# kpreid/all-is-cubes

Measured on NVIDIA H100. Metric: Mrays/s, higher is better.
Workload: dtype f64 geometry / f32 colour

## Files before the change

### all-is-cubes_b200/aicb200/__init__.py

```python
from __future__ import annotations

import ctypes as C
import dataclasses
import math
import os
from typing import Optional, Sequence

import numpy as np

from . import abi
from .abi import (FOG_ABRUPT, FOG_COMPROMISE, FOG_NONE, FOG_PHYSICAL, LIGHT_BOUNCE, LIGHT_COARSE, LIGHT_FLAT, LIGHT_LINEAR,
                  LIGHT_NONE, LIGHT_SMOOTHSTEP, TONE_CLAMP, TONE_REINHARD, TRANSPARENCY_SURFACE,
                  TRANSPARENCY_THRESHOLD, TRANSPARENCY_VOLUMETRIC)

PKG_DIR = os.path.dirname(os.path.dirname(os.path.abspath(__file__)))
LIB_PATH = os.environ.get("AICB200_LIB") or os.path.join(PKG_DIR, "libaicb200.so")
LIGHT_RAY_DTYPE = np.dtype(abi.LightRay)


class AicbError(RuntimeError):
    def __init__(self, status: int, message: str):
        super().__init__(f"{abi.STATUS_NAMES.get(status, status)}: {message}")
        self.status = status

# ... 787 lines not shown
    for c in rgb:
        f = np.float32(c) / np.float32(255.0)
        if f <= np.float32(0.04045):
            out.append(float(np.float32(f * np.float32(25.0 / 323.0))))
        else:
            x = np.float32(np.float32(200.0) * f + np.float32(11.0)) / np.float32(211.0)
            out.append(float(np.float32(float(x) ** float(np.float32(12.0 / 5.0)))))
    return tuple(out)


class Context:
    _default = None

    def __init__(self, device_id: int = -1):
        lib = load_library()
        self.handle = C.c_void_p()
        _check(lib.aicb_ctx_create(device_id, C.byref(self.handle)))
        self.device_id = lib.aicb_ctx_device(self.handle)
        self._pending = None

    def settle(self):
        if self._pending is not None:
            self._pending.result()

    @classmethod
    def default(cls) -> "Context":
        if cls._default is None:
            cls._default = Context(-1)
        return cls._default

    def derive_block_light(self, blocks: Sequence[Block]) -> list:
        if not blocks:
            return []
        descs = _block_descs(blocks)
        out = (abi.BlockLight * len(blocks))()
        _check(load_library().aicb_derive_block_light(self.handle, descs, len(blocks), out))
        return [BlockLight.from_abi(o) for o in out]

    def close(self):
        if self.handle:
            load_library().aicb_ctx_destroy(self.handle)
            self.handle = C.c_void_p()


@dataclasses.dataclass
class RenderInfo:
    cubes_traced: int
    rays: int
    algorithmic_bytes: int
    counters: tuple
    kernel_ms: float
    flaws: int
    stage_ms: tuple = (0.0, 0.0, 0.0, 0.0)

    @staticmethod
    def from_abi(i: abi.RenderInfo) -> "RenderInfo":
        return RenderInfo(int(i.cubes_traced), int(i.rays), int(i.algorithmic_bytes), tuple(int(c) for c in i.counters),
                          float(i.kernel_ms), int(i.flaws), tuple(float(v) for v in i.stage_ms))


@dataclasses.dataclass
class Rendering:
    size: tuple
    data: np.ndarray
    flaws: int
    info: RenderInfo


def _torch():
    import torch
    return torch


def _ctx_device(ctx: "Context"):
    return _torch().device("cuda", ctx.device_id)


def _device_outputs(out, device, spec) -> dict:
    torch = _torch()
    given = out if isinstance(out, dict) else ({next(iter(spec)): out} if out is not None else {})
    unknown = set(given) - set(spec)
    if unknown:
        raise ValueError(f"out= names outputs this call does not make: {sorted(unknown)}")
    tensors = {}
    for name, (shape, dtype) in spec.items():
        t = given.get(name)
        if t is None:
            t = torch.empty(shape, dtype=dtype, device=device)
        elif tuple(t.shape) != tuple(shape) or t.dtype != dtype or t.device != device or not t.is_contiguous():
            raise ValueError(f"out[{name!r}] must be a contiguous {dtype} tensor of shape {tuple(shape)} on {device}, "
                             f"not {t.dtype} {tuple(t.shape)} on {t.device}")
        tensors[name] = t
    return tensors


def _outs_abi(n: int, tensors: dict) -> abi.DeviceOutputs:
    o = abi.DeviceOutputs()
    for name, t in tensors.items():
        setattr(o, name, t.data_ptr())
    o.len = n
    return o


def _stream(device) -> int:
    return _torch().cuda.current_stream(device).cuda_stream or 1


class DeviceRendering:

    def __init__(self, scene, issue, build):
        self._scene = scene
# ... 1180 lines not shown
```

### all-is-cubes_b200/aicb200/abi.py

```python
import ctypes as C

import numpy as np

ABI_VERSION = 27

BLOCKS_DERIVE_LIGHT = 1

OK, ERR_INVALID, ERR_OOM, ERR_CUDA, ERR_UNSUPPORTED, ERR_BUSY, ERR_RETRY = range(7)
STATUS_NAMES = {0: "OK", 1: "ERR_INVALID", 2: "ERR_OOM", 3: "ERR_CUDA", 4: "ERR_UNSUPPORTED", 5: "ERR_BUSY", 6: "ERR_RETRY"}

FACE_WITHIN, FACE_NX, FACE_NY, FACE_NZ, FACE_PX, FACE_PY, FACE_PZ = range(7)
FOG_NONE, FOG_ABRUPT, FOG_COMPROMISE, FOG_PHYSICAL = range(4)
LIGHT_NONE, LIGHT_FLAT, LIGHT_COARSE, LIGHT_LINEAR, LIGHT_SMOOTHSTEP, LIGHT_BOUNCE = range(6)
TRANSPARENCY_SURFACE, TRANSPARENCY_VOLUMETRIC, TRANSPARENCY_THRESHOLD = range(3)
TONE_CLAMP, TONE_REINHARD = range(2)


class Aab(C.Structure):
    _fields_ = [("lower", C.c_int32 * 3), ("size", C.c_uint32 * 3)]


class Voxel(C.Structure):
    _fields_ = [("rgba", C.c_float * 4), ("emission", C.c_float * 3), ("flags", C.c_uint32)]

# ... 37 lines not shown
        ("block_ids", C.c_void_p),
        ("light", C.c_void_p),
        ("blocks", C.POINTER(BlockDesc)),
        ("n_blocks", C.c_size_t),
        ("sky", Sky),
        ("light_max_distance", C.c_uint8),
        ("_pad", C.c_uint8 * 7),
    ]


class CameraData(C.Structure):
    _fields_ = [
        ("inverse_projection_view", C.c_double * 16),
        ("fb_width", C.c_uint32),
        ("fb_height", C.c_uint32),
        ("exposure", C.c_float),
        ("_pad", C.c_uint32),
    ]


CAMERA_DTYPE = np.dtype([("inverse_projection_view", "<f8", (16,)), ("fb_width", "<u4"), ("fb_height", "<u4"),
                         ("exposure", "<f4"), ("_pad", "<u4")])
assert CAMERA_DTYPE.itemsize == C.sizeof(CameraData) == 144


class Options(C.Structure):
    _fields_ = [
        ("fog", C.c_uint8),
        ("lighting_display", C.c_uint8),
        ("transparency", C.c_uint8),
        ("antialiasing_always", C.c_uint8),
        ("tone_mapping", C.c_uint8),
        ("debug_pixel_cost", C.c_uint8),
        ("include_sky", C.c_uint8),
        ("bounce_samples", C.c_uint8),
        ("transparency_threshold", C.c_float),
        ("maximum_intensity", C.c_float),
        ("view_distance", C.c_double),
    ]


class Shard(C.Structure):
    _fields_ = [("strip_rows", C.c_uint32), ("index", C.c_uint32), ("count", C.c_uint32)]


class RenderInfo(C.Structure):
    _fields_ = [
        ("cubes_traced", C.c_uint64),
        ("rays", C.c_uint64),
        ("algorithmic_bytes", C.c_uint64),
        ("counters", C.c_uint64 * 6),
        ("kernel_ms", C.c_float),
        ("flaws", C.c_uint16),
        ("_pad", C.c_uint16),
        ("stage_ms", C.c_float * 4),
    ]


class Hit(C.Structure):
    _fields_ = [("cube", C.c_int32 * 3), ("voxel", C.c_int32 * 3), ("resolution", C.c_int32), ("face", C.c_int32)]


class LightRay(C.Structure):
    _fields_ = [("trigger_cube", C.c_int32 * 3), ("value_cube", C.c_int32 * 3), ("value", C.c_uint8 * 4),
                ("light_from_struck_face", C.c_float * 3), ("_pad", C.c_uint32)]


class LightUpdatesInfo(C.Structure):
    _fields_ = [("update_count", C.c_uint64), ("queue_count", C.c_uint64), ("max_update_difference", C.c_uint8),
                ("max_queue_priority", C.c_uint8), ("_pad", C.c_uint8 * 6)]


class Layer(C.Structure):
    _fields_ = [("scene", C.c_void_p), ("camera", C.POINTER(CameraData)), ("options", C.POINTER(Options))]


class GroupLayer(C.Structure):
    _fields_ = [("scene", C.c_void_p), ("camera", C.POINTER(CameraData)), ("options", C.POINTER(Options))]


TEXT_ENTERED_SPACE, TEXT_EMPTY, TEXT_INCOMPLETE, TEXT_BLANK = -1, -2, -3, -4
LAYER_NONE, LAYER_WORLD, LAYER_UI = 0, 1, 2


class TerminalPixel(C.Structure):
    _fields_ = [("rgba", C.c_float * 4), ("text", C.c_int32), ("layer", C.c_int32)]


class DeviceOutputs(C.Structure):
    _fields_ = [("srgb8", C.c_void_p), ("rgba16f", C.c_void_p), ("colorbuf", C.c_void_p), ("depth", C.c_void_p),
                ("hit", C.c_void_p), ("steps", C.c_void_p), ("text", C.c_void_p), ("texel_rgba16f", C.c_void_p),
                ("texel_depth", C.c_void_p), ("terminal", C.c_void_p), ("len", C.c_size_t), ("full_frame", C.c_uint32),
                ("_pad", C.c_uint32)]


TEXTURE_INCREMENTAL, TEXTURE_CONSISTENT = 1, 2


class TextureTargetInfo(C.Structure):
    _fields_ = [("width", C.c_uint32), ("height", C.c_uint32), ("strategy", C.c_uint32), ("_pad", C.c_uint32),
                ("dirty_pixels", C.c_uint64), ("next_pick", C.c_uint64), ("cycle_length", C.c_uint64)]


VOXEL_NOT_SELECTABLE = 1
VOXEL_NO_COLLISION = 2
BLOCK_NOT_SELECTABLE = 1
CURSOR_NONE = 0xFFFFFFFF
# ... 220 lines not shown
```

### all-is-cubes_b200/csrc/aicb200.cu

```cuda
#include <algorithm>
#include <array>
#include <cmath>
#include <cstdio>
#include <cstdlib>
#include <cstring>
#include <initializer_list>
#include <mutex>
#include <string>
#include <unordered_map>
#include <vector>

#include <cuda_runtime.h>
#include <cub/device/device_radix_sort.cuh>

#include "block_words.cuh"
#include "brick_room.h"
#include "host_tables.h"
#include "internal.h"

using namespace aicb;

static thread_local std::string g_last_error = "";

aicb_status aicb_fail(aicb_status st, const std::string &msg) {
// ... 516 lines not shown
    P.lighting = opt->lighting_display;
    P.transparency = opt->transparency;
    P.threshold = opt->transparency_threshold;
    P.antialias = (cam && opt->antialiasing_always) ? 1 : 0;
    if (cam && out.force_antialias >= 0) P.antialias = (uint32_t)out.force_antialias;
    P.tone_mapping = opt->tone_mapping;
    P.maximum_intensity = opt->maximum_intensity;
    P.view_distance = opt->view_distance;
    P.debug_pixel_cost = opt->debug_pixel_cost;
    P.include_sky = opt->include_sky;
    P.out_full_frame = out.full_frame ? 1 : 0;
    P.target = out.target;
    const int tgt = out.kind;
    if (tgt == TGT_VIEWS) P.target.view_tiles = P.tiles_x * P.tiles_y;
    P.counters = ctx->d_counters.get<unsigned long long>();
    P.task_counter = ctx->d_tile_counter;
    P.refill_threshold = REFILL_THRESHOLD;
    P.tail_divisor = TAIL_DIVISOR;
    P.event_threshold = EVENT_THRESHOLD;

    uint64_t frame_pixels = pixels, frame_rays = pixels * (P.antialias ? 4 : 1);
    uint64_t out_bytes =
        (P.target.out_srgb8 ? 4 : (tgt == TGT_TEX ? 12 : (tgt == TGT_TERM ? 24 : (P.target.out_rgba16f ? 8 : 16)))) * pixels;
    if (continues && ctx->last_scene) {
        aicb_scene *prev = ctx->last_scene;
        frame_pixels += prev->pending_pixels;
        frame_rays += prev->pending_rays;
        out_bytes += prev->pending_out_bytes;
        prev->pending = false;
    }
    sc->pending = true;
    sc->pending_pixels = frame_pixels;
    sc->pending_rays = frame_rays;
    sc->pending_out_bytes = out_bytes;

    P.n_samples = P.antialias ? 4 : 1;
    const bool fused = (opt->lighting_display == AICB_LIGHT_NONE || opt->lighting_display == AICB_LIGHT_FLAT) &&
                       !ctx->deep_frames;
    const uint64_t total_tasks = (uint64_t)P.n_tasks * P.n_samples;
    uint64_t CHUNK = (uint64_t)4 << 20;
    {
        const uint64_t per_task = sizeof(RayRecordA) + sizeof(RayRecordB) + sizeof(TaskOut) + 4 * N_BINS +
                                  (uint64_t)ctx->hits_per_task * (sizeof(HitRecord) + (fused ? 0 : sizeof(ShadedHit)));
        uint64_t fit = ((uint64_t)8 << 30) / per_task;
        if (fit < (1u << 17)) fit = 1u << 17;
        if (fit < CHUNK) CHUNK = fit & ~(uint64_t)127;
    }
    const uint64_t chunk_cap = total_tasks < CHUNK ? total_tasks : CHUNK;
    uint64_t cap = chunk_cap * ctx->hits_per_task;
    if (cap < (1u << 16)) cap = 1u << 16;
    if (cap > 0xfffffff0ull) cap = 0xfffffff0ull;
    cap &= ~(uint64_t)(HIT_CHUNK - 1);
    P.hit_capacity = (uint32_t)cap;
    TRY(ctx->primary.size(chunk_cap, P.hit_capacity, !fused));
    ctx->primary.bind(P, chunk_cap, !fused);
    P.ray_counter = ctx->d_tile_counter + 2;
    sc->pending_fused = fused;
    P.hit_counter = ctx->d_tile_counter + 1;
    P.bin_count = ctx->d_tile_counter + 4;
    P.bin_stride = (uint32_t)chunk_cap;
    P.overflow_flag = (unsigned int *)(P.counters + 7);
    if (stream != ctx->stream.get()) CU(cudaStreamWaitEvent(stream, ctx->ev_delta.get(), 0));
    if (ctx->frame_in_flight && ctx->last_stream != stream) CU(cudaStreamWaitEvent(stream, ctx->ev1.get(), 0));
    ctx->frame_in_flight = true;
    ctx->last_stream = stream;
    ctx->last_scene = sc;
    if (continues) {
        CU(cudaMemsetAsync(ctx->d_tile_counter, 0, 2 * (4 + N_BINS) * sizeof(unsigned int), stream));
    } else {
        CU(cudaMemsetAsync(P.counters, 0, 8 * sizeof(unsigned long long) + 2 * (4 + N_BINS) * sizeof(unsigned int), stream));
        CU(cudaEventRecord(ctx->ev0.get(), stream));
    }
    if (total_tasks > 0) {
        const bool volumetric = opt->transparency == AICB_TRANSPARENCY_VOLUMETRIC;
        const int lc = opt->lighting_display == AICB_LIGHT_NONE ? LC_NONE
                       : (opt->lighting_display == AICB_LIGHT_FLAT ? LC_FLAT
                          : (opt->lighting_display == AICB_LIGHT_BOUNCE ? LC_BOUNCE : LC_INTERP));
        TraceParams Q;
        const bool bounce = lc == LC_BOUNCE;
        if (bounce) {
            TRY(ctx->secondary.size(chunk_cap, P.hit_capacity, true));
            TRY(ctx->d_bounce.ensure(chunk_cap * 104 + 256));
            char *b = ctx->d_bounce.get<char>();
            P.bounce_mode = BOUNCE_PRIMARY;
            P.bounce_samples = opt->bounce_samples;
            P.bounce_rays = (double *)b;
            P.bounce_rng = (unsigned long long *)(b + chunk_cap * 48);
            P.bounce_sum = (float4 *)(b + chunk_cap * 80);
            P.bounce_req = (uint32_t *)(b + chunk_cap * 96);
            P.ray_index = (uint32_t *)(b + chunk_cap * 100);
            Q = P;
            Q.ray_index = nullptr;
            Q.bounce_mode = BOUNCE_SECONDARY;
            Q.rays = P.bounce_rays;
            Q.tiles_y = 1;
            Q.shard_count = 1; Q.shard_index = 0; Q.strip_rows = 1;
            Q.antialias = 0;
            Q.n_samples = 1;
            Q.task_base = 0;
            Q.lighting = AICB_LIGHT_FLAT;
            Q.include_sky = 1;
            Q.exposure = 1.0f;
            Q.out_full_frame = 0;
            Q.target = {};
            ctx->secondary.bind(Q, chunk_cap, true);
            Q.task_counter = ctx->d_tile_counter + (4 + N_BINS);
            Q.hit_counter = Q.task_counter + 1;
            Q.ray_counter = Q.task_counter + 2;
// ... 83 lines not shown
        float t[4] = {0, 0, 0, 0};
        for (int i = 0; i < (sc->pending_fused ? 3 : 4); i++) cudaEventElapsedTime(&t[i], ctx->ev_k[i].get(), ctx->ev_k[i + 1].get());
        if (ctx->d_debug && ctx->debug_warps) {
            std::vector<unsigned long long> w(4 * (size_t)ctx->debug_warps);
            cudaMemcpy(w.data(), ctx->d_debug.get(), w.size() * 8, cudaMemcpyDeviceToHost);
            unsigned long long t0 = ~0ull, t1 = 0, passes = 0, rays = 0;
            for (uint32_t i = 0; i < ctx->debug_warps; i++) { t0 = std::min(t0, w[4 * i]); t1 = std::max(t1, w[4 * i + 1]); passes += w[4 * i + 2]; rays += w[4 * i + 3]; }
            std::vector<double> ends;
            for (uint32_t i = 0; i < ctx->debug_warps; i++) ends.push_back((double)(w[4 * i + 1] - t0) * 1e-6);
            std::sort(ends.begin(), ends.end());
            auto q = [&](double f) { return ends[(size_t)(f * (ends.size() - 1))]; };
            fprintf(stderr, "[aicb200] march warps %u: end times ms min %.3f p10 %.3f p50 %.3f p90 %.3f p99 %.3f max %.3f; passes/warp %.0f rays %llu\n",
                    ctx->debug_warps, q(0), q(0.1), q(0.5), q(0.9), q(0.99), q(1.0), (double)passes / ctx->debug_warps, rays);
        }
        if (sc->pending_fused)
            fprintf(stderr, "[aicb200] gen %.3f ms  march %.3f ms  resolve (shade + encode) %.3f ms  (hits %llu)\n", t[0], t[1],
                    t[2], c[3]);
        else
            fprintf(stderr, "[aicb200] gen %.3f ms  march %.3f ms  shade %.3f ms  encode %.3f ms  (hits %llu)\n", t[0], t[1], t[2],
                    t[3], c[3]);
    }
    if (sc->pending_rays) ctx->deep_frames = c[3] * 4 >= sc->pending_rays * 3;
    if (c[7]) {
        if (ctx->hits_per_task >= 2048)
            return fail(AICB_ERR_OOM, "hit stream overflowed at its largest capacity (2048 hit records per ray)");
        ctx->hits_per_task *= 4;
        ctx->shallow_frames = 0;
        return fail(AICB_ERR_RETRY, "hit stream overflowed; its capacity has been raised - re-issue the render");
    }
    if (ctx->hits_per_task > 8 && c[3] * 16 < (unsigned long long)sc->pending_rays * ctx->hits_per_task) {
        if (++ctx->shallow_frames >= 16) {
            ctx->hits_per_task /= 4;
            ctx->shallow_frames = 0;
            ctx->primary.release_hits();
            ctx->secondary.release_hits();
        }
    } else {
        ctx->shallow_frames = 0;
    }
    if (info) {
        std::memset(info, 0, sizeof *info);
        float ms = 0.0f;
        CU(cudaEventElapsedTime(&ms, ctx->ev0.get(), ctx->ev1.get()));
        info->kernel_ms = ms;
        if (sc->pending_rays && ctx->stage_timing)
            for (int i = 0; i < (sc->pending_fused ? 3 : 4); i++)
                cudaEventElapsedTime(&info->stage_ms[i], ctx->ev_k[i].get(), ctx->ev_k[i + 1].get());
        info->cubes_traced = c[0];
        info->rays = sc->pending_rays;
        for (int i = 0; i < 5; i++) info->counters[i] = c[1 + i];
        info->counters[5] = sc->pending_pixels;
        info->algorithmic_bytes = 2 * c[1] + 2 * c[2] + 32 * c[3] + 4 * c[4] + 32 * c[5] + sc->pending_out_bytes;
        info->flaws = 0;
    }
    sc->pending = false;
    return AICB_OK;
}

aicb_status issue_empty_frame(aicb_scene *s, const aicb_options *opt, cudaStream_t stream) {
    return launch_trace(s, nullptr, opt, nullptr, Outputs{}, stream);
}

aicb_status check_device_pointer(const void *p, int device, bool peer_ok, size_t align, const char *what) {
    if ((uintptr_t)p % align)
        return fail(AICB_ERR_INVALID, std::string(what) + " is not aligned to " + std::to_string(align) + " bytes");
    cudaPointerAttributes a;
    const cudaError_t e = cudaPointerGetAttributes(&a, p);
    if (e != cudaSuccess) cudaGetLastError();
    if (e != cudaSuccess || (a.type != cudaMemoryTypeDevice && a.type != cudaMemoryTypeManaged))
        return fail(AICB_ERR_INVALID, std::string(what) + " is not device memory");
    if (a.device == device) return AICB_OK;
    int can = 0;
    if (peer_ok && cudaDeviceCanAccessPeer(&can, device, a.device) == cudaSuccess && can) return AICB_OK;
    return fail(AICB_ERR_INVALID, std::string(what) + " is memory of another device");
}

aicb_status output_target(const aicb_device_outputs *d, DeviceCall call, bool need_colorbuf, Outputs *o) {
    if (!d) return fail(AICB_ERR_INVALID, "outs is NULL");
    const void *const ptr[10] = {d->srgb8, d->rgba16f, d->colorbuf, d->depth, d->hit,
                                 d->steps, d->text,    d->texel_rgba16f, d->texel_depth, d->terminal};
    unsigned set = 0;
    for (int i = 0; i < 10; i++)
        if (ptr[i]) set |= 1u << i;
    const unsigned SRGB8 = 1, RGBA16F = 2, AUX = 4 | 8 | 16 | 32, TEXT = 64, TEXELS = 128 | 256, TERMINAL = 512;
    const bool aux = set && !(set & ~AUX);
    bool ok = false;
    switch (call) {
        case DEV_FRAME: ok = set == SRGB8 || set == RGBA16F || aux || set == TEXT; break;
        case DEV_RAYS: ok = aux; break;
        case DEV_LAYERS: ok = set == SRGB8 || set == TERMINAL || set == TEXELS; break;
    }
    if (set == 0 && d->len == 0) ok = true;
    if (!ok) return fail(AICB_ERR_INVALID, "the outputs are not a set that this call gives (aicb_device_outputs)");
    if (aux && need_colorbuf && d->len && !d->colorbuf) return fail(AICB_ERR_INVALID, "colorbuf is NULL");
    TargetParams &t = o->target;
    t.out_srgb8 = (uchar4 *)d->srgb8;
    t.out_text = d->text;
    o->aux = aux;
    if (aux) {
        t.out_colorbuf = (float4 *)d->colorbuf;
        t.out_depth = d->depth;
        t.out_hit = d->hit;
        t.out_steps = d->steps;
    }
    if (set == RGBA16F) t.out_rgba16f = (uint2 *)d->rgba16f;
    if (set == TEXELS) {
// ... 1777 lines not shown
    const aicb_device_outputs o = one_output(&aicb_device_outputs::text, out, out_len);
    return on_scene(s, [&](Replicas r) { return views_host(r, cameras, n_views, opt, o, STAGE_GIVEN, info); });
}

aicb_status aicb_render_views_device(aicb_scene *s, const aicb_camera *d_cameras, size_t n_views, uint32_t fb_width,
                                     uint32_t fb_height, const aicb_options *opt, const aicb_device_outputs *outs,
                                     void *stream) {
    if (!s || !outs) return fail(AICB_ERR_INVALID, "NULL argument");
    if (outs->full_frame) return fail(AICB_ERR_INVALID, "full_frame is for aicb_render_device");
    TRY(check_views(d_cameras, false, n_views, &fb_width, &fb_height, opt, outs->len));
    std::lock_guard<std::mutex> lock(s->ctx->mu);
    CU(cudaSetDevice(s->ctx->device));
    Outputs o;
    TRY(device_target(outs, s->ctx->device, DEV_FRAME, false, false, &o));
    if (n_views) TRY(check_device_pointer(d_cameras, s->ctx->device, false, 8, "the camera table"));
    cudaStream_t st = stream ? (cudaStream_t)stream : s->ctx->stream.get();
    if (outs->len == 0) return issue_empty_frame(s, opt, st);
    views_part(&o, d_cameras, n_views, 0, 1);
    const aicb_camera size = views_frame_camera(fb_width, fb_height);
    return launch_trace(s, &size, opt, nullptr, o, st);
}

aicb_status aicb_check_layers(const aicb_layer *world, const aicb_layer *ui, const float *no_world_rgba, size_t out_len,
                              const aicb_layer **lead_out) {
    const bool have_world = world && world->scene, have_ui = ui && ui->scene;
    if (!have_world && !have_ui && !no_world_rgba) return fail(AICB_ERR_INVALID, "no layer to draw");
    const aicb_layer *lead = have_world ? world : ui;
    if (!lead || !lead->camera || !lead->options) return fail(AICB_ERR_INVALID, "a layer needs its camera and options");
    if (have_ui && (!ui->camera || !ui->options)) return fail(AICB_ERR_INVALID, "a layer needs its camera and options");
    if (have_world && have_ui) {
        if (world->scene->ctx != ui->scene->ctx) return fail(AICB_ERR_INVALID, "the layers must live on one context");
        if (world->camera->fb_width != ui->camera->fb_width || world->camera->fb_height != ui->camera->fb_height)
            return fail(AICB_ERR_INVALID, "the layers' cameras must share the framebuffer size");
    }
    aicb_status st = aicb_check_render_args(lead->scene, lead->camera, lead->options, nullptr, out_len);
    if (st != AICB_OK) return st;
    if (have_ui && have_world) {
        st = validate_options(ui->options);
        if (st != AICB_OK) return st;
    }
    *lead_out = lead;
    return AICB_OK;
}

void aicb_merge_info(aicb_render_info *sum, const aicb_render_info *one, bool same_part) {
    auto time = [same_part](float t, float u) { return same_part ? t + u : std::max(t, u); };
    sum->cubes_traced += one->cubes_traced;
    sum->rays += one->rays;
    sum->algorithmic_bytes += one->algorithmic_bytes;
    for (int k = 0; k < 6; k++) sum->counters[k] += one->counters[k];
    sum->kernel_ms = time(sum->kernel_ms, one->kernel_ms);
    for (int k = 0; k < 4; k++) sum->stage_ms[k] = time(sum->stage_ms[k], one->stage_ms[k]);
    sum->flaws |= one->flaws;
}

aicb_status aicb_trace_pass(FramePart *parts, size_t n_parts, const aicb_camera *cam, const aicb_options *opt,
                            bool want_info, const std::vector<Delivery> &copies) {
    std::vector<size_t> todo(n_parts), again;
    for (size_t i = 0; i < n_parts; i++) todo[i] = i;
    while (!todo.empty()) {
        std::vector<aicb_ctx *> round = {parts[0].scene->ctx};
        for (size_t i : todo) {
            const FramePart &p = parts[i];
            aicb_ctx *ctx = p.scene->ctx;
            CU(cudaSetDevice(ctx->device));
            aicb_status r = launch_trace(p.scene, cam, opt, p.shard, p.out, ctx->stream.get());
            if (r != AICB_OK) return r;
            if (i) round.push_back(ctx);
        }
        if (!copies.empty()) TRY(deliver(round.data(), round.size(), copies));
        again.clear();
        for (size_t i : todo) {
            aicb_scene *sc = parts[i].scene;
            CU(cudaSetDevice(sc->ctx->device));
            CU(cudaStreamSynchronize(sc->ctx->stream.get()));
            aicb_render_info one{};
            aicb_status r = finish(sc, want_info ? &one : nullptr);
            if (r == AICB_ERR_RETRY) { again.push_back(i); continue; }
            if (r != AICB_OK) return r;
            aicb_merge_info(&parts[i].info, &one, true);
        }
        todo.swap(again);
    }
    return AICB_OK;
}

aicb_status aicb_trace_layers(const aicb_layer *world, const aicb_layer *ui, const float *backdrop_rgba,
                              const float *no_world_rgba, LayerPart *parts, size_t n_parts,
                              const std::vector<Delivery> &copies, aicb_render_info *total, cudaStream_t async) {
    const bool have_world = world && world->scene, have_ui = ui && ui->scene;
    const aicb_layer *lead = have_world ? world : ui;
    aicb_status st = AICB_OK;
    const int aa = lead->options->antialiasing_always ? 1 : 0;
    auto n_tasks = [&](const LayerPart &p) -> size_t {
        return (listed(p.out.target) ? (size_t)p.out.target.n_list
                                        : (((size_t)lead->camera->fb_width + TILE_W - 1) / TILE_W) *
                                              ((shard_rows(lead->camera->fb_height, &p.shard) + TILE_H - 1) / TILE_H) * 32) *
               (aa ? 4 : 1);
    };
    float backdrop[4] = {0, 0, 0, 1}, no_world[4] = {0, 0, 0, 0};
    const bool have_backdrop = backdrop_rgba && !(backdrop_rgba[0] == 0.0f && backdrop_rgba[1] == 0.0f &&
                                                   backdrop_rgba[2] == 0.0f && backdrop_rgba[3] == 0.0f);
    if (have_backdrop) {
        for (int i = 0; i < 3; i++) backdrop[i] = backdrop_rgba[i] * backdrop_rgba[3];
        backdrop[3] = 1.0f - backdrop_rgba[3];
    }
// ... 351 lines not shown
```

### all-is-cubes_b200/csrc/internal.h

```cpp
#pragma once
#include <memory>
#include <mutex>
#include <string>
#include <utility>
#include <vector>

#include <cuda_runtime.h>

#include "trace_kernel.cuh"

aicb_status aicb_fail(aicb_status st, const std::string &msg);
aicb_status aicb_cuda_fail(cudaError_t e, const char *what);
#define CU(call)                                                   \
    do {                                                           \
        cudaError_t e__ = (call);                                  \
        if (e__ != cudaSuccess) return aicb_cuda_fail(e__, #call); \
    } while (0)
#define TRY(call)                                  \
    do {                                           \
        aicb_status st__ = (call);                 \
        if (st__ != AICB_OK) return st__;          \
    } while (0)

struct DeviceMemory {
    static cudaError_t alloc(void **p, size_t bytes) { return cudaMalloc(p, bytes); }
    static void release(void *p) { cudaFree(p); }
};
struct PinnedMemory {
    static cudaError_t alloc(void **p, size_t bytes) { return cudaMallocHost(p, bytes); }
    static void release(void *p) { cudaFreeHost(p); }
};

template <typename Memory>
class Buffer {
public:
    Buffer() = default;
    Buffer(Buffer &&o) noexcept : p_(std::exchange(o.p_, nullptr)), bytes_(std::exchange(o.bytes_, 0)) {}
    Buffer &operator=(Buffer &&o) noexcept {
        if (this != &o) {
            reset();
            p_ = std::exchange(o.p_, nullptr);
            bytes_ = std::exchange(o.bytes_, 0);
        }
        return *this;
    }
    ~Buffer() { reset(); }

    aicb_status ensure(size_t bytes) {
        if (bytes_ >= bytes) return AICB_OK;
        reset();
        void *p = nullptr;
        CU(Memory::alloc(&p, bytes));
        p_ = p;
// ... 16 lines not shown
    }

    template <typename T = void>
    T *get() const { return static_cast<T *>(p_); }
    size_t bytes() const { return bytes_; }
    explicit operator bool() const { return p_ != nullptr; }

private:
    void *p_ = nullptr;
    size_t bytes_ = 0;
};
using DeviceBuffer = Buffer<DeviceMemory>;
using PinnedBuffer = Buffer<PinnedMemory>;

struct EventDestroy {
    void operator()(cudaEvent_t e) const { cudaEventDestroy(e); }
};
struct StreamDestroy {
    void operator()(cudaStream_t s) const { cudaStreamDestroy(s); }
};
using Event = std::unique_ptr<CUevent_st, EventDestroy>;
using Stream = std::unique_ptr<CUstream_st, StreamDestroy>;

inline aicb_status create_event(Event &e, unsigned int flags) {
    cudaEvent_t raw = nullptr;
    CU(cudaEventCreateWithFlags(&raw, flags));
    e.reset(raw);
    return AICB_OK;
}

inline uint32_t cell_word(uint32_t id, uint8_t kind, bool wide) { return id | ((uint32_t)kind << (wide ? 16 : 14)); }

struct ChunkStreams {
    DeviceBuffer rays, task_out, hits, shaded, bin_list;

    aicb_status size(uint64_t chunk_cap, uint32_t hit_capacity, bool shade) {
        TRY(rays.ensure(chunk_cap * (sizeof(aicb::RayRecordA) + sizeof(aicb::RayRecordB)) + 16));
        TRY(task_out.ensure(chunk_cap * sizeof(aicb::TaskOut) + 16));
        TRY(hits.ensure((size_t)hit_capacity * sizeof(aicb::HitRecord) + 64));
        if (shade) TRY(shaded.ensure((size_t)hit_capacity * sizeof(aicb::ShadedHit) + 64));
        return bin_list.ensure((size_t)aicb::N_BINS * chunk_cap * 4 + 64);
    }
    void bind(aicb::TraceParams &P, uint64_t chunk_cap, bool shade) const {
        P.rays_a = rays.get<aicb::RayRecordA>();
        P.rays_b = (aicb::RayRecordB *)(rays.get<char>() + chunk_cap * sizeof(aicb::RayRecordA));
        P.task_out = task_out.get<aicb::TaskOut>();
        P.hits = hits.get<aicb::HitRecord>();
        P.shaded = shade ? shaded.get<aicb::ShadedHit>() : nullptr;
        P.bin_list = bin_list.get<uint32_t>();
    }
    void release_hits() {
        hits.reset();
        shaded.reset();
    }
};

struct LightChart {
    DeviceBuffer pre, chains, node_rel, euler, term_scratch;
    uint32_t nodes = 0, n_chains = 0, n_euler = 0, walk_blocks = 0;
};

struct LightState {
    struct Own {
        DeviceBuffer sky_term;
        DeviceBuffer overflow;
        DeviceBuffer overflow_count;
    } own;
    struct Shared {
        DeviceBuffer pending;
        DeviceBuffer tile_max;
        DeviceBuffer step;
        DeviceBuffer list, new_light, diff;
        DeviceBuffer counters;
        DeviceBuffer changes;
        DeviceBuffer dirty, push_targets;
    } shared;

    aicb_status ensure(aicb_scene *s, size_t replica, size_t n_replicas, const std::vector<float4> *terms);

    uint32_t *changed() const { return own.overflow.get<uint32_t>(); }
    uint32_t *chunk_sums() const { return shared.diff.get<uint32_t>(); }
    uint32_t *taken_indices() const { return shared.list.get<uint32_t>(); }
    uint32_t *taken_texels() const { return shared.new_light.get<uint32_t>(); }
};

struct aicb_ctx {
    int device = 0;
    int num_sms = 0;
    Stream stream;
    Event ev0, ev1;
    Event ev_light[2];
    Event ev_join;
    Event ev_k[5];
    bool profile_kernels = false;
    bool stage_timing = true;
    PinnedBuffer h_delta;
    DeviceBuffer d_delta;
    Event ev_delta;
    DeviceBuffer d_debug;
    uint32_t debug_warps = 0;
    DeviceBuffer d_counters;
    unsigned int *d_tile_counter = nullptr;
    DeviceBuffer d_lut;
    DeviceBuffer d_out, d_aux;
    ChunkStreams primary, secondary;
    DeviceBuffer d_bounce;
    uint32_t hits_per_task = 8;
    uint32_t shallow_frames = 0;
    bool deep_frames = false;
    PinnedBuffer h_stage;
    bool frame_in_flight = false;
    cudaStream_t last_stream = nullptr;
    struct aicb_scene *last_scene = nullptr;
    DeviceBuffer d_task_aux;
    DeviceBuffer d_task_depth;
    DeviceBuffer d_task_text;
    LightChart light_chart;
    DeviceBuffer d_derive;
    DeviceBuffer d_inputs;
    DeviceBuffer d_cursor;
    DeviceBuffer d_bodies;
    DeviceBuffer d_exposure;
    PinnedBuffer h_views;
    DeviceBuffer d_views;
    std::mutex mu;
};

struct BlockTable {
    struct Extent {
        uint32_t brick_off, n_bricks;
        uint32_t pal_off, n_pal;
    };

    DeviceBuffer blocks;
    DeviceBuffer blk_tab;
    DeviceBuffer light;
    DeviceBuffer bricks;
    DeviceBuffer palette;
    DeviceBuffer pal_tab;

    void bind(aicb::DeviceScene &ds) const {
        ds.blocks = blocks.get<aicb::BlockRec>();
        ds.blk_tab = blk_tab.get<float4>();
        ds.bricks = bricks.get<uint16_t>();
        ds.palette = palette.get<float4>();
        ds.pal_tab = pal_tab.get<float2>();
    }
};

struct SpaceHost {
    size_t volume = 0;
    std::vector<uint16_t> h_ids;
    bool ids_stale = false;
    std::vector<uint8_t> kind;
    std::vector<BlockTable::Extent> extent;
    size_t n_bricks = 0, n_palette = 0;
    size_t dead_bricks = 0, dead_pal = 0;
    bool wide_bricks = false;
    uint32_t light_max_distance = 0;
    uint64_t light_stats[4] = {0, 0, 0, 0};

    size_t block_count() const { return kind.size(); }
// ... 310 lines not shown
```

### all-is-cubes_b200/csrc/trace_kernel.cuh

```cuda
#pragma once
#include <cstdint>
#include <type_traits>
#include <cuda_runtime.h>

#include "../../include/aicb200.h"

#ifdef __CUDACC__
#include <cuda_fp16.h>
#include "exact_math.cuh"
#endif

struct LightBlockDev {
    float face_color[7][4];
    float emission[3];
    uint32_t flags;
};
static_assert(sizeof(LightBlockDev) == 128, "LightBlockDev must be 128 bytes");

namespace aicb {

constexpr uint32_t KIND_SINGLE = 0;
constexpr uint32_t KIND_RECURSIVE = 1;
constexpr uint32_t KIND_INVISIBLE = 2;

// ... 108 lines not shown
            double *out_task_depth;
            float *out_tex_depth;
        };
        struct {
            aicb_terminal_pixel *out_term;
            const int2 *in_text;
            int2 *out_task_text;
            int32_t text_start;
        };
        struct {
            const aicb_camera *cameras;
            uint32_t view_tiles;
            uint32_t view_first, view_step;
        };
    };
};

struct TraceParams {
    DeviceScene scene;
    double m[16];
    uint32_t fb_width, fb_height;
    double inv_width, inv_height;
    float exposure;
    uint32_t fog;
    uint32_t lighting;
    uint32_t transparency;
    float threshold;
    uint32_t antialias;
    uint32_t tone_mapping;
    float maximum_intensity;
    double view_distance;
    uint32_t debug_pixel_cost;
    uint32_t include_sky;
    uint32_t local_rows;
    uint32_t strip_rows, shard_index, shard_count;
    const double *rays;
    uint64_t n_rays;
    uint32_t tiles_x, tiles_y;
    uint32_t n_tasks;
    uint32_t out_full_frame;
    uint32_t n_samples;
    uint32_t task_base;
    RayRecordA *rays_a;
    RayRecordB *rays_b;
    unsigned int *ray_counter;
    uint32_t *ray_index;
    TaskOut *task_out;
    HitRecord *hits;
    ShadedHit *shaded;
    unsigned int *hit_counter;
    uint32_t *bin_list;
    unsigned int *bin_count;
    uint32_t bin_stride;
    unsigned int *overflow_flag;
    uint32_t hit_capacity;
    uint32_t event_threshold;
    uint32_t tail_divisor;
    uint32_t refill_threshold;
    TargetParams target;
    uint32_t bounce_mode;
    uint32_t bounce_samples;
    uint32_t bounce_pass;
    uint32_t *bounce_req;
    unsigned long long *bounce_rng;
    float4 *bounce_sum;
    double *bounce_rays;
    unsigned long long *counters;
    unsigned int *task_counter;
    unsigned long long *debug_warp_times;
};

#ifdef __CUDACC__

#define AICB_DEV __device__ __forceinline__
#define AICB_NOINLINE static __device__ __noinline__

constexpr int LC_NONE = 0, LC_FLAT = 1, LC_INTERP = 2, LC_BOUNCE = 3;
constexpr uint32_t BOUNCE_OFF = 0, BOUNCE_PRIMARY = 1, BOUNCE_SECONDARY = 2;
constexpr int TILE_W = 8, TILE_H = 4;
constexpr int WARPS_PER_BLOCK = 4;
constexpr int N_BINS = 8;
constexpr uint32_t HIT_CHUNK = 8;
constexpr uint32_t HIT_NONE = 0xffffffffu;
constexpr int MIN_BLOCKS_PER_SM = 5;
constexpr uint32_t EVENT_THRESHOLD = 24, TAIL_DIVISOR = 2, REFILL_THRESHOLD = 4;


constexpr double D_INF = __builtin_huge_val();

__device__ __forceinline__ void grid_dependency_sync() {
    asm volatile("griddepcontrol.launch_dependents;" ::: "memory");
    asm volatile("griddepcontrol.wait;" ::: "memory");
}

struct Ray {
    double ox, oy, oz, dx, dy, dz;
    double tdx, tdy, tdz;
    double half_over_len;
    int sx, sy, sz;
};

struct Caster {
    double tmx, tmy, tmz;
    double last_t;
    int rx, ry, rz;
    int face;
// ... 464 lines not shown
    return P.target.view_first + (pixel_task >> 5) / P.target.view_tiles * P.target.view_step;
}
template <bool LIST, bool VIEWS = false>
AICB_DEV bool task_pixel(const TraceParams &P, uint32_t pixel_task, uint32_t *px, uint32_t *py, size_t *out_index) {
    if (!VIEWS && P.rays) {
        *px = *py = 0;
        *out_index = pixel_task;
        return pixel_task < P.n_rays;
    }
    if (LIST && P.target.n_list) {
        if (pixel_task >= P.target.n_list) return false;
        const bool picked = P.target.picks != PICK_LIST;
        const uint32_t v = picked ? pick_pixel(P.target.picks, P.target.pixel_list, P.target.pick_central, P.fb_width,
                                               P.fb_height, P.target.pick_base + pixel_task)
                                  : __ldg(P.target.pixel_list + pixel_task);
        *px = v % P.fb_width;
        *py = v / P.fb_width;
        *out_index = picked ? v : pixel_task;
        return true;
    }
    const uint32_t tile = VIEWS ? (pixel_task >> 5) % P.target.view_tiles : pixel_task >> 5, in_tile = pixel_task & 31;
    const uint32_t tx = tile % P.tiles_x, ty = tile / P.tiles_x;
    const uint32_t x = tx * TILE_W + (in_tile & (TILE_W - 1));
    const uint32_t ly = ty * TILE_H + (in_tile / TILE_W);
    uint32_t y = ly;
    if (P.shard_count > 1) {
        const uint32_t strip_local = ly / P.strip_rows;
        y = (strip_local * P.shard_count + P.shard_index) * P.strip_rows + ly % P.strip_rows;
    }
    *px = x;
    *py = y;
    *out_index = VIEWS ? ((size_t)task_view(P, pixel_task) * P.fb_height + y) * P.fb_width + x
                       : (P.out_full_frame ? (size_t)y * P.fb_width + x : (size_t)ly * P.fb_width + x);
    return x < P.fb_width && ly < P.local_rows;
}

template <bool VIEWS>
AICB_DEV void gen_rays(const TraceParams &P, uint32_t n_chunk_tasks) {
    grid_dependency_sync();
    const uint32_t i = blockIdx.x * blockDim.x + threadIdx.x;
    const bool in_range = i < n_chunk_tasks;
    const uint32_t task = P.task_base + i;
    const uint32_t pixel_task = task / P.n_samples, sample = task % P.n_samples;
    RayRecordA rec;
    RayRecordB rb;
    uint32_t px, py;
    size_t out_index;
    bool active = in_range && task_pixel<!VIEWS, VIEWS>(P, pixel_task, &px, &py, &out_index);
    if (P.bounce_mode == BOUNCE_SECONDARY && active) active = P.bounce_req[i] != HIT_NONE;
    rec.flags = 0;
    bool running = false;
    uint32_t octant = 0;
    int bin = 0;
    if (active) {
        const DeviceScene &S = P.scene;
        double o[3], d[3];
        if (P.rays) {
            const double *rp = P.rays + 6 * (size_t)pixel_task;
            o[0] = rp[0]; o[1] = rp[1]; o[2] = rp[2]; d[0] = rp[3]; d[1] = rp[4]; d[2] = rp[5];
        } else {
            const double *m = VIEWS ? P.target.cameras[task_view(P, pixel_task)].inverse_projection_view : P.m;
            pixel_ray(P, m, px, py, P.n_samples == 4 ? (int)sample : -1, o, d);
        }
        octant = ((d[0] >= 0.0) << 2) + ((d[1] >= 0.0) << 1) + (d[2] >= 0.0);
        const double d_orig[3] = {d[0], d[1], d[2]};
        if (!((fabs(d[0]) < 1e100) & (fabs(d[1]) < 1e100) & (fabs(d[2]) < 1e100))) { d[0] = d[1] = d[2] = 0.0; }
    if (!certainly_misses(o, d, S)) {
        rec.t_to_abs = sqrt(d_orig[0] * d_orig[0] + d_orig[1] * d_orig[1] + d_orig[2] * d_orig[2]);
        rec.t_to_view = (float)(rec.t_to_abs / P.view_distance);
        Ray r;
        r.ox = o[0]; r.oy = o[1]; r.oz = o[2];
        r.dx = d[0]; r.dy = d[1]; r.dz = d[2];
        r.sx = signum_101(d[0]); r.sy = signum_101(d[1]); r.sz = signum_101(d[2]);
        r.tdx = 1.0 / fabs(d[0]); r.tdy = 1.0 / fabs(d[1]); r.tdz = 1.0 / fabs(d[2]);
        r.half_over_len = 0.5 / sqrt(d[0] * d[0] + d[1] * d[1] + d[2] * d[2]);
        Level lv;
        lv.lox = S.lo[0]; lv.loy = S.lo[1]; lv.loz = S.lo[2];
        lv.nx = S.size[0]; lv.ny = S.size[1]; lv.nz = S.size[2];
        lv.base = 0;
        Caster c;
        c.tmx = c.tmy = c.tmz = c.last_t = 0.0;
        c.rx = c.ry = c.rz = 0;
        c.face = 0;
        c.idx = 0;
        bool valid;
        running = caster_begin(c, r, o[0], o[1], o[2], lv, &valid);
        rec.ox = r.ox; rec.oy = r.oy; rec.oz = r.oz; rec.dx = r.dx; rec.dy = r.dy; rec.dz = r.dz;
        rb.tdx = r.tdx; rb.tdy = r.tdy; rb.tdz = r.tdz;
        rb.half_over_len = r.half_over_len;
        rb.tmx = c.tmx; rb.tmy = c.tmy; rb.tmz = c.tmz; rb.last_t = c.last_t;
        rb.rx = c.rx; rb.ry = c.ry; rb.rz = c.rz;
        rb.task = i;
        rec.flags = ((uint32_t)c.face & 7u) | (running ? 8u : 0u) | (valid ? 16u : 0u) | 32u | ((uint32_t)(r.sx + 1) << 6) |
                    ((uint32_t)(r.sy + 1) << 8) | ((uint32_t)(r.sz + 1) << 10) | (octant << 12);
        if (running) {
            const float lo3[3] = {(float)lv.lox, (float)lv.loy, (float)lv.loz};
            const float n3[3] = {(float)lv.nx, (float)lv.ny, (float)lv.nz};
            float tn = 0.0f, tf = 3.0e38f, l1 = 0.0f;
#pragma unroll
            for (int a = 0; a < 3; a++) {
                const float da = (float)d[a], oa = (float)o[a];
                if (da != 0.0f) {
                    const float t0 = (lo3[a] - oa) / da, t1 = (lo3[a] + n3[a] - oa) / da;
                    tn = fmaxf(tn, fminf(t0, t1));
                    tf = fminf(tf, fmaxf(t0, t1));
                    l1 += fabsf(da);
                }
            }
            const float crossings = fmaxf(tf - tn, 0.0f) * l1;
            const float frac = crossings / (n3[0] + n3[1] + n3[2]);
            int q = (int)(frac * (float)N_BINS);
            q = q < 0 ? 0 : (q > N_BINS - 1 ? N_BINS - 1 : q);
            bin = N_BINS - 1 - q;
        }
    }
    }
    const unsigned listed = __ballot_sync(0xffffffffu, running);
    if (running) {
        const int lane = (int)(threadIdx.x & 31);
        const unsigned below = listed & ((1u << lane) - 1u);
        uint32_t rbase = 0;
        if (below == 0) rbase = atomicAdd(P.ray_counter, (unsigned)__popc(listed));
        rbase = __shfl_sync(listed, rbase, __ffs(listed) - 1);
        const uint32_t r = rbase + __popc(below);
        const unsigned peers = __match_any_sync(listed, bin);
        const int leader = __ffs(peers) - 1;
        uint32_t base = 0;
        if (lane == leader) base = atomicAdd(P.bin_count + bin, (unsigned)__popc(peers));
        base = __shfl_sync(peers, base, leader);
        const uint32_t slot = base + __popc(peers & ((1u << lane) - 1u));
        P.bin_list[(size_t)bin * P.bin_stride + slot] = r;
        if (P.ray_index) P.ray_index[i] = r;
        const uint4 *src = reinterpret_cast<const uint4 *>(&rec);
        uint4 *dst = reinterpret_cast<uint4 *>(P.rays_a + r);
#pragma unroll
        for (int k = 0; k < 4; k++) st_stream(dst + k, src[k]);
        src = reinterpret_cast<const uint4 *>(&rb);
        dst = reinterpret_cast<uint4 *>(P.rays_b + r);
#pragma unroll
        for (int k = 0; k < 5; k++) st_stream(dst + k, src[k]);
    } else if (in_range) {
        TaskOut o;
        o.first_hit = 0xffffffffu;
        o.steps = 0;
        o.flags = octant;
        o.n_hits = 0;
        *reinterpret_cast<uint4 *>(P.task_out + i) = *reinterpret_cast<const uint4 *>(&o);
    }
}
static __global__ void __launch_bounds__(128) gen_kernel(const __grid_constant__ TraceParams P, uint32_t n_chunk_tasks) {
    gen_rays<false>(P, n_chunk_tasks);
}
static __global__ void __launch_bounds__(128) gen_views_kernel(const __grid_constant__ TraceParams P,
                                                               uint32_t n_chunk_tasks) {
    gen_rays<true>(P, n_chunk_tasks);
}

template <bool VOLUMETRIC, bool WIDE, bool AUX, bool BRICK_WIDE>
__global__ void __launch_bounds__(WARPS_PER_BLOCK * 32, AUX ? 1 : MIN_BLOCKS_PER_SM)
trace_kernel(const __grid_constant__ TraceParams P, uint32_t n_chunk_tasks) {
    grid_dependency_sync();
    const DeviceScene &S = P.scene;
    const int lane = threadIdx.x & 31;
    constexpr float F_NEG_INF = -__builtin_huge_valf();
    constexpr int COUNTER_STATIC = 0x3fffffff;

    unsigned long long n_outer = 0, n_inner = 0, n_blocks = 0;

// ... 1185 lines not shown
```

### bindings/rust/all-is-cubes-b200-sys/src/lib.rs

```rust
#![allow(non_camel_case_types)]
#![no_std]

use core::ffi::{c_char, c_int, c_void};

pub type aicb_status = c_int;
pub const AICB_OK: aicb_status = 0;
pub const AICB_ERR_INVALID: aicb_status = 1;
pub const AICB_ERR_OOM: aicb_status = 2;
pub const AICB_ERR_CUDA: aicb_status = 3;
pub const AICB_ERR_UNSUPPORTED: aicb_status = 4;
pub const AICB_ERR_BUSY: aicb_status = 5;
pub const AICB_ERR_RETRY: aicb_status = 6;

pub const AICB_BLOCKS_DERIVE_LIGHT: u32 = 1;

pub const AICB_TEXT_ENTERED_SPACE: i32 = -1;
pub const AICB_TEXT_EMPTY: i32 = -2;
pub const AICB_TEXT_INCOMPLETE: i32 = -3;
pub const AICB_TEXT_BLANK: i32 = -4;

pub const AICB_LAYER_NONE: i32 = 0;
pub const AICB_LAYER_WORLD: i32 = 1;
pub const AICB_LAYER_UI: i32 = 2;

// ... 154 lines not shown
    pub bounds: aicb_aab,
    pub block_ids: *const u16,
    pub light: *const [u8; 4],
    pub blocks: *const aicb_block_desc,
    pub n_blocks: usize,
    pub sky: aicb_sky,
    pub light_max_distance: u8,
    pub _pad: [u8; 7],
}

#[repr(C)]
#[derive(Clone, Copy, Debug)]
pub struct aicb_camera {
    pub inverse_projection_view: [f64; 16],
    pub fb_width: u32,
    pub fb_height: u32,
    pub exposure: f32,
    pub _pad: u32,
}

#[repr(C)]
#[derive(Clone, Copy, Debug)]
pub struct aicb_options {
    pub fog: u8,
    pub lighting_display: u8,
    pub transparency: u8,
    pub antialiasing_always: u8,
    pub tone_mapping: u8,
    pub debug_pixel_cost: u8,
    pub include_sky: u8,
    pub bounce_samples: u8,
    pub transparency_threshold: f32,
    pub maximum_intensity: f32,
    pub view_distance: f64,
}

#[repr(C)]
#[derive(Clone, Copy, Debug, Default)]
pub struct aicb_shard {
    pub strip_rows: u32,
    pub index: u32,
    pub count: u32,
}

#[repr(C)]
#[derive(Clone, Copy, Debug, Default)]
pub struct aicb_render_info {
    pub cubes_traced: u64,
    pub rays: u64,
    pub algorithmic_bytes: u64,
    pub counters: [u64; 6],
    pub kernel_ms: f32,
    pub flaws: u16,
    pub _pad: u16,
    pub stage_ms: [f32; 4],
}

#[repr(C)]
#[derive(Clone, Copy, Debug, Default)]
pub struct aicb_hit {
    pub cube: [i32; 3],
    pub voxel: [i32; 3],
    pub resolution: i32,
    pub face: i32,
}

#[repr(C)]
#[derive(Clone, Copy, Debug, Default)]
pub struct aicb_light_ray {
    pub trigger_cube: [i32; 3],
    pub value_cube: [i32; 3],
    pub value: [u8; 4],
    pub light_from_struck_face: [f32; 3],
    pub _pad: u32,
}

#[repr(C)]
#[derive(Clone, Copy, Debug, Default)]
pub struct aicb_light_updates_info {
    pub update_count: u64,
    pub queue_count: u64,
    pub max_update_difference: u8,
    pub max_queue_priority: u8,
    pub _pad: [u8; 6],
}

#[repr(C)]
#[derive(Clone, Copy, Debug, Default)]
pub struct aicb_terminal_pixel {
    pub rgba: [f32; 4],
    pub text: i32,
    pub layer: i32,
}

#[repr(C)]
pub struct aicb_ctx {
    _opaque: [u8; 0],
}
#[repr(C)]
pub struct aicb_scene {
    _opaque: [u8; 0],
}
#[repr(C)]
pub struct aicb_group {
    _opaque: [u8; 0],
}
#[repr(C)]
// ... 421 lines not shown
```

### include/aicb200.h

```cpp
#ifndef AICB200_H
#define AICB200_H

#include <stddef.h>
#include <stdint.h>

#ifdef __cplusplus
extern "C" {
#endif

#define AICB_ABI_VERSION 27

typedef enum aicb_status {
    AICB_OK = 0,
    AICB_ERR_INVALID = 1,
    AICB_ERR_OOM = 2,
    AICB_ERR_CUDA = 3,
    AICB_ERR_UNSUPPORTED = 4,
    AICB_ERR_BUSY = 5,
    AICB_ERR_RETRY = 6
} aicb_status;


typedef struct aicb_aab {
    int32_t lower[3];
// ... 34 lines not shown
} aicb_sky;

typedef struct aicb_scene_desc {
    aicb_aab bounds;
    const uint16_t *block_ids;
    const uint8_t (*light)[4];
    const aicb_block_desc *blocks;
    size_t n_blocks;
    aicb_sky sky;
    uint8_t light_max_distance;
    uint8_t _pad[7];
} aicb_scene_desc;

typedef struct aicb_camera {
    double inverse_projection_view[16];
    uint32_t fb_width, fb_height;
    float exposure;
    uint32_t _pad;
} aicb_camera;

enum { AICB_FOG_NONE = 0, AICB_FOG_ABRUPT = 1, AICB_FOG_COMPROMISE = 2, AICB_FOG_PHYSICAL = 3 };
enum { AICB_LIGHT_NONE = 0, AICB_LIGHT_FLAT = 1, AICB_LIGHT_COARSE = 2, AICB_LIGHT_LINEAR = 3,
       AICB_LIGHT_SMOOTHSTEP = 4, AICB_LIGHT_BOUNCE = 5  };
enum { AICB_TRANSPARENCY_SURFACE = 0, AICB_TRANSPARENCY_VOLUMETRIC = 1, AICB_TRANSPARENCY_THRESHOLD = 2 };
enum { AICB_TONE_CLAMP = 0, AICB_TONE_REINHARD = 1 };

typedef struct aicb_options {
    uint8_t fog;
    uint8_t lighting_display;
    uint8_t transparency;
    uint8_t antialiasing_always;
    uint8_t tone_mapping;
    uint8_t debug_pixel_cost;
    uint8_t include_sky;
    uint8_t bounce_samples;
    float transparency_threshold;
    float maximum_intensity;
    double view_distance;
} aicb_options;

typedef struct aicb_shard {
    uint32_t strip_rows;
    uint32_t index;
    uint32_t count;
} aicb_shard;

typedef struct aicb_render_info {
    uint64_t cubes_traced;
    uint64_t rays;
    uint64_t algorithmic_bytes;
    uint64_t counters[6];
    float kernel_ms;
    uint16_t flaws;
    uint16_t _pad;
    float stage_ms[4];
} aicb_render_info;

#define AICB_TEXT_ENTERED_SPACE (-1)
#define AICB_TEXT_EMPTY (-2)
#define AICB_TEXT_INCOMPLETE (-3)
#define AICB_TEXT_BLANK (-4)

typedef struct aicb_hit {
    int32_t cube[3];
    int32_t voxel[3];
    int32_t resolution;
    int32_t face;
} aicb_hit;

typedef struct aicb_ctx aicb_ctx;
typedef struct aicb_scene aicb_scene;

uint32_t aicb_abi_version(void);
aicb_status aicb_ctx_create(int device_id, aicb_ctx **out);
void aicb_ctx_destroy(aicb_ctx *);
aicb_status aicb_ctx_stage_timing(aicb_ctx *, int enable);
int aicb_ctx_device(const aicb_ctx *);
const char *aicb_last_error(void);

typedef struct aicb_block_light {
    float face_colors[6][4];
    float color[4];
    float emission[3];
    uint8_t opaque_faces;
    uint8_t visible;
    uint8_t _pad[2];
} aicb_block_light;
aicb_status aicb_derive_block_light(aicb_ctx *, const aicb_block_desc *descs, size_t n, aicb_block_light *out);

aicb_status aicb_scene_create(aicb_ctx *, const aicb_scene_desc *, aicb_scene **out);
aicb_status aicb_scene_update_cubes(aicb_scene *, const int32_t (*cubes)[3], const uint16_t *block_ids,
                                    const uint8_t (*light)[4], size_t n);
aicb_status aicb_scene_update_region(aicb_scene *, const aicb_aab *region, const uint16_t *block_ids_or_null,
                                     uint16_t uniform_id, const uint8_t (*light_or_null)[4]);
aicb_status aicb_scene_update_blocks(aicb_scene *, const uint16_t *indices, const aicb_block_desc *descs, size_t n);
aicb_status aicb_scene_append_blocks(aicb_scene *, const aicb_block_desc *descs, size_t n);
aicb_status aicb_scene_fill_uniform(aicb_scene *, const aicb_block_desc *block);
aicb_status aicb_scene_upload_light(aicb_scene *, const uint8_t (*light)[4], size_t n_texels);
void aicb_scene_destroy(aicb_scene *);
uint64_t aicb_scene_device_bytes(const aicb_scene *);
aicb_status aicb_scene_set_physics(aicb_scene *, const aicb_sky *sky, uint8_t light_max_distance);

aicb_status aicb_scene_update_cubes_device(aicb_scene *, const int32_t (*d_cubes)[3], const uint16_t *d_ids,
                                           const uint8_t (*d_light_or_null)[4], size_t n, void *stream);
aicb_status aicb_scene_update_region_device(aicb_scene *, const aicb_aab *region, const uint16_t *d_ids_or_null,
                                            uint16_t uniform_id, const uint8_t (*d_light_or_null)[4], void *stream);
aicb_status aicb_scene_upload_light_device(aicb_scene *, const uint8_t (*d_light)[4], size_t n_texels, void *stream);
// ... 457 lines not shown
```

Measured before the change: 2793.

## Bin rays by previous frame's per-ray step counts when the view repeats

When scene, camera matrix, framebuffer and shard settings exactly match the previous frame, rays are binned by the step count each ray recorded last frame. Each warp takes the maximum cost, falls back to a chord-length estimate when that is zero, and maps its log2 to a bin, instead of using the geometric chord fraction. The goal is to group rays of similar traversal cost so warps diverge less and the trace is better load-balanced. The cost is a key comparison per frame, an extra read of the old task output, and warp reductions. The gain depends on frame-to-frame coherence, and the path only turns on for repeated identical views. A ray_order flag is added to the render info to report when the ordering was used.

After: 2981 (median of 6 runs). +6.7%, better.

```diff
diff --git a/all-is-cubes_b200/aicb200/__init__.py b/all-is-cubes_b200/aicb200/__init__.py
--- a/all-is-cubes_b200/aicb200/__init__.py
+++ b/all-is-cubes_b200/aicb200/__init__.py
@@ -863,11 +863,12 @@
     kernel_ms: float
     flaws: int
     stage_ms: tuple = (0.0, 0.0, 0.0, 0.0)
+    ray_order: int = 0
 
     @staticmethod
     def from_abi(i: abi.RenderInfo) -> "RenderInfo":
         return RenderInfo(int(i.cubes_traced), int(i.rays), int(i.algorithmic_bytes), tuple(int(c) for c in i.counters),
-                          float(i.kernel_ms), int(i.flaws), tuple(float(v) for v in i.stage_ms))
+                          float(i.kernel_ms), int(i.flaws), tuple(float(v) for v in i.stage_ms), int(i.ray_order))
 
 
 @dataclasses.dataclass
diff --git a/all-is-cubes_b200/aicb200/abi.py b/all-is-cubes_b200/aicb200/abi.py
--- a/all-is-cubes_b200/aicb200/abi.py
+++ b/all-is-cubes_b200/aicb200/abi.py
@@ -113,7 +113,7 @@
         ("counters", C.c_uint64 * 6),
         ("kernel_ms", C.c_float),
         ("flaws", C.c_uint16),
-        ("_pad", C.c_uint16),
+        ("ray_order", C.c_uint16),
         ("stage_ms", C.c_float * 4),
     ]
 
diff --git a/all-is-cubes_b200/csrc/aicb200.cu b/all-is-cubes_b200/csrc/aicb200.cu
--- a/all-is-cubes_b200/csrc/aicb200.cu
+++ b/all-is-cubes_b200/csrc/aicb200.cu
@@ -592,8 +592,25 @@
     if (cap > 0xfffffff0ull) cap = 0xfffffff0ull;
     cap &= ~(uint64_t)(HIT_CHUNK - 1);
     P.hit_capacity = (uint32_t)cap;
+    RayOrderKey key;
+    if (cam && tgt != TGT_VIEWS && !listed(out.target) && opt->lighting_display != AICB_LIGHT_BOUNCE &&
+        total_tasks > 0 && total_tasks <= CHUNK) {
+        key.scene = sc;
+        std::memcpy(key.view, cam->inverse_projection_view, sizeof key.view);
+        key.fb_width = P.fb_width;
+        key.fb_height = P.fb_height;
+        key.n_samples = P.n_samples;
+        key.strip_rows = P.strip_rows;
+        key.shard_index = P.shard_index;
+        key.shard_count = P.shard_count;
+    }
+    const bool order_by_steps = key.scene && key == ctx->order_key;
+    ctx->order_key = RayOrderKey{};
     TRY(ctx->primary.size(chunk_cap, P.hit_capacity, !fused));
     ctx->primary.bind(P, chunk_cap, !fused);
+    P.order_by_steps = order_by_steps ? 1 : 0;
+    ctx->order_key = key;
+    ctx->ray_ordered = (continues && ctx->ray_ordered) || order_by_steps;
     P.ray_counter = ctx->d_tile_counter + 2;
     sc->pending_fused = fused;
     P.hit_counter = ctx->d_tile_counter + 1;
@@ -783,6 +800,7 @@
         info->counters[5] = sc->pending_pixels;
         info->algorithmic_bytes = 2 * c[1] + 2 * c[2] + 32 * c[3] + 4 * c[4] + 32 * c[5] + sc->pending_out_bytes;
         info->flaws = 0;
+        info->ray_order = ctx->ray_ordered ? 1 : 0;
     }
     sc->pending = false;
     return AICB_OK;
@@ -2666,6 +2684,7 @@
     sum->kernel_ms = time(sum->kernel_ms, one->kernel_ms);
     for (int k = 0; k < 4; k++) sum->stage_ms[k] = time(sum->stage_ms[k], one->stage_ms[k]);
     sum->flaws |= one->flaws;
+    sum->ray_order |= one->ray_order;
 }
 
 aicb_status aicb_trace_pass(FramePart *parts, size_t n_parts, const aicb_camera *cam, const aicb_options *opt,
diff --git a/all-is-cubes_b200/csrc/internal.h b/all-is-cubes_b200/csrc/internal.h
--- a/all-is-cubes_b200/csrc/internal.h
+++ b/all-is-cubes_b200/csrc/internal.h
@@ -1,4 +1,5 @@
 #pragma once
+#include <cstring>
 #include <memory>
 #include <mutex>
 #include <string>
@@ -121,6 +122,18 @@
     void release_hits() {
         hits.reset();
         shaded.reset();
+    }
+};
+
+struct RayOrderKey {
+    const aicb_scene *scene = nullptr;
+    double view[16] = {};
+    uint32_t fb_width = 0, fb_height = 0, n_samples = 0;
+    uint32_t strip_rows = 0, shard_index = 0, shard_count = 0;
+    bool operator==(const RayOrderKey &o) const {
+        return scene == o.scene && std::memcmp(view, o.view, sizeof view) == 0 && fb_width == o.fb_width &&
+               fb_height == o.fb_height && n_samples == o.n_samples && strip_rows == o.strip_rows &&
+               shard_index == o.shard_index && shard_count == o.shard_count;
     }
 };
 
@@ -177,6 +190,8 @@
     uint32_t hits_per_task = 8;
     uint32_t shallow_frames = 0;
     bool deep_frames = false;
+    RayOrderKey order_key;
+    bool ray_ordered = false;
     PinnedBuffer h_stage;
     bool frame_in_flight = false;
     cudaStream_t last_stream = nullptr;
diff --git a/all-is-cubes_b200/csrc/trace_kernel.cuh b/all-is-cubes_b200/csrc/trace_kernel.cuh
--- a/all-is-cubes_b200/csrc/trace_kernel.cuh
+++ b/all-is-cubes_b200/csrc/trace_kernel.cuh
@@ -184,6 +184,7 @@
     uint32_t *bin_list;
     unsigned int *bin_count;
     uint32_t bin_stride;
+    uint32_t order_by_steps;
     unsigned int *overflow_flag;
     uint32_t hit_capacity;
     uint32_t event_threshold;
@@ -754,6 +755,7 @@
     bool running = false;
     uint32_t octant = 0;
     int bin = 0;
+    uint32_t cost = 0, chord_cost = 0;
     if (active) {
         const DeviceScene &S = P.scene;
         double o[3], d[3];
@@ -810,12 +812,23 @@
                 }
             }
             const float crossings = fmaxf(tf - tn, 0.0f) * l1;
-            const float frac = crossings / (n3[0] + n3[1] + n3[2]);
-            int q = (int)(frac * (float)N_BINS);
-            q = q < 0 ? 0 : (q > N_BINS - 1 ? N_BINS - 1 : q);
-            bin = N_BINS - 1 - q;
-        }
-    }
+            if (P.order_by_steps) {
+                cost = min(__ldg(&P.task_out[i].steps), 1u << 30);
+                chord_cost = (uint32_t)fminf(crossings, 1073741824.0f);
+            } else {
+                const float frac = crossings / (n3[0] + n3[1] + n3[2]);
+                int q = (int)(frac * (float)N_BINS);
+                q = q < 0 ? 0 : (q > N_BINS - 1 ? N_BINS - 1 : q);
+                bin = N_BINS - 1 - q;
+            }
+        }
+    }
+    }
+    if (P.order_by_steps) {
+        uint32_t m = __reduce_max_sync(0xffffffffu, running ? cost : 0u);
+        if (m == 0) m = __reduce_max_sync(0xffffffffu, running ? chord_cost : 0u);
+        const int cls = 31 - __clz((int)(m + 1u));
+        bin = N_BINS - 1 - (cls > N_BINS - 1 ? N_BINS - 1 : cls);
     }
     const unsigned listed = __ballot_sync(0xffffffffu, running);
     if (running) {
diff --git a/bindings/rust/all-is-cubes-b200-sys/src/lib.rs b/bindings/rust/all-is-cubes-b200-sys/src/lib.rs
--- a/bindings/rust/all-is-cubes-b200-sys/src/lib.rs
+++ b/bindings/rust/all-is-cubes-b200-sys/src/lib.rs
@@ -230,7 +230,7 @@
     pub counters: [u64; 6],
     pub kernel_ms: f32,
     pub flaws: u16,
-    pub _pad: u16,
+    pub ray_order: u16,
     pub stage_ms: [f32; 4],
 }
 
diff --git a/include/aicb200.h b/include/aicb200.h
--- a/include/aicb200.h
+++ b/include/aicb200.h
@@ -110,7 +110,7 @@
     uint64_t counters[6];
     float kernel_ms;
     uint16_t flaws;
-    uint16_t _pad;
+    uint16_t ray_order;
     float stage_ms[4];
 } aicb_render_info;
 
```
